# byteowlz/kokorox

Measured on NVIDIA B200. Metric: audio-seconds per second, higher is better.
Workload: dtype bf16

## Files before the change

kokorox_b200/csrc/kernels.h:

```cpp
#pragma once
#include "common.h"
#include <cuda_bf16.h>

namespace kkx {

enum Act : int { ACT_NONE = 0, ACT_LRELU = 1, ACT_SNAKE = 2, ACT_GELU_NEW = 3 };

struct ConvArgs {
  const float* in = nullptr; int ldi = 0;
  const int* in_off = nullptr; const int* in_len = nullptr;
  const int* m_len = nullptr; int max_m = 0; int B = 1;
  long long sum_m = 0;
  const float* w = nullptr; const float* bias = nullptr;
  int Ci = 0, Co = 0, ks = 1, dil = 1, pad = 0, stride = 1;
  const float* pscale = nullptr; const float* pshift = nullptr; int pld = 0;
  int pact = ACT_NONE; float pslope = 0.f; const float* palpha = nullptr;
  float* out = nullptr; int ldo = 0; int ocol = 0; const int* out_off = nullptr;
  int ors = 1, oro = 0;
  int eact = ACT_NONE;
  const float* res = nullptr; int ldr = 0; int rcol = 0; const int* res_off = nullptr;
  int res_shift = 0;
  float oscale = 1.f; int accumulate = 0;
};
void launch_conv_f32(const ConvArgs& a, cudaStream_t st);
// ... 54 lines not shown
void launch_im2col_bf16(const float* in, int ldi, int C, int ks, int stride, int pad, void* out, int Cpad,
                        int rows_total, const int* in_off, const int* in_len, const int* out_off,
                        const int* out_len, int B, int max_out_len, cudaStream_t st, int force_generic = 0);
void launch_pool_up_bf16(const float* in, int ldi, const float* scale, const float* shift, float slope,
                         const float* w, const float* bias, int C, void* out, int Cpad, int rows_total,
                         const int* in_off, const int* in_len, const int* out_off, int B, int max_len,
                         cudaStream_t st);

struct ArbConvArgs {
  const void* x = nullptr; int in_bf16 = 0;
  const float* scale = nullptr; const float* shift = nullptr;
  const float* alpha = nullptr;
  const void* tmB = nullptr;
  int C = 0, ks = 1, dil = 1, pad = 0;
  const int* off = nullptr; const int* len = nullptr;
  const int* tile_start = nullptr;
  int B = 1; int total_tiles = 0; long long sum_m = 0;
  const float* bias = nullptr;
  __nv_bfloat16* out_bf16 = nullptr;
  float* out_f32 = nullptr;
  const float* res = nullptr; float oscale = 1.f; int accumulate = 0;
  int res_bf16 = 0;
  float* part = nullptr; int nchunk = 0;
  long long* timing = nullptr;
  int debug = 0;
  int post = 0, cout = 0, ldo = 0; float slope = 0.f;
};
int arb_tile_rows(int C, int ks);
bool arb_conv_supported(int C, int ks, int dil, int B);
void launch_arb_conv(const ArbConvArgs& a, cudaStream_t st);
// ... 115 lines not shown
```

kokorox_b200/csrc/kernels_arb.cu:

```cuda
#include "kernels.h"
#include "tc_ptx.cuh"
#include <type_traits>
#include <cstdlib>

namespace kkx {

namespace {

#ifdef KKX_ARB_TIMING
#define TIM_DECL(n) long long tim_acc[n] = {0}; long long tim_last = clock64(); const bool tim_on = a.timing && blockIdx.x == 0
#define TICK(slot) do { if (tim_on) { const long long now_ = clock64(); tim_acc[slot] += now_ - tim_last; tim_last = now_; } } while (0)
#define TIM_FLUSH(base, n) do { if (tim_on) for (int i_ = 0; i_ < (n); i_++) atomicAdd(reinterpret_cast<unsigned long long*>(a.timing) + (base) + i_, (unsigned long long)tim_acc[i_]); } while (0)
#else
#define TIM_DECL(n)
#define TICK(slot)
#define TIM_FLUSH(base, n)
#endif

#ifdef KKX_EXPERIMENTS
#define ARB_DBG(a, bit) ((a).debug & (bit))
#else
#define ARB_DBG(a, bit) (0)
#endif

constexpr int kArbThreads = 512;
constexpr int kArbMaxB = 512;

template <int BN, int MSUB, bool T>
struct ArbCfg {
  static constexpr int KCH = BN / 64;
  static constexpr int RA = MSUB * 128 + 56;
  static constexpr uint32_t A_SLOT = RA * 128;
  static constexpr int NA = (BN == 128 && (!T || MSUB == 4)) ? 2 : 3;
  static constexpr uint32_t B_STAGE = BN * 128;
  static constexpr int NB = (T && MSUB == 4) ? 4 : (BN == 128) ? 6 : 3;
  static constexpr int PITCH = 36;
  static constexpr uint32_t STG = T ? 0 : 2 * 128 * PITCH * 4;
  static constexpr uint32_t STAT = 4 * BN * 2 * 4;
  static constexpr uint32_t COEF = 3 * BN * 4;
  static constexpr int NBAR = 2 * NA + 2 * NB + 4;
  static constexpr uint32_t SMEM = NA * A_SLOT + NB * B_STAGE + STG + STAT + COEF + NBAR * 8 + 16 + (3 * kArbMaxB + 2) * 4 + 1024;
  static_assert(A_SLOT % 1024 == 0, "A slot must keep the 1024-byte swizzle alignment");
};

__device__ __forceinline__ uint32_t pack_bf16(float lo, float hi) {
  __nv_bfloat162 p = __floats2bfloat162_rn(lo, hi);
  return *reinterpret_cast<uint32_t*>(&p);
}

struct TileCur {
  int b, mt;
  __device__ __forceinline__ void init(const int* ts, int B, int tile) {
    int lo = 0, hi = B;
    while (hi - lo > 1) {
      const int mid = (lo + hi) >> 1;
      if (ts[mid] <= tile) lo = mid; else hi = mid;
    }
    b = lo; mt = tile - ts[lo];
  }
  __device__ __forceinline__ void next(const int* ts) {
    mt++;
    while (ts[b] + mt >= ts[b + 1]) { b++; mt = 0; if (ts[b] < 0) break; }
  }
};

template <int BN, int MSUB, bool CONV2, bool T, bool POST = false, int SB = 0, bool PB = false>
__global__ void __launch_bounds__(kArbThreads, 1) arb_conv_kernel(const __grid_constant__ CUtensorMap tmB, ArbConvArgs a) {
  static_assert(SB == 0 || (!POST && (CONV2 || SB == 1)), "stream-bf16 variants: conv1 SB=1, conv2 SB=1 (bf16 out) / SB=2 (fp32 out)");
  static_assert(!PB || (T && !CONV2 && !POST && SB == 0 && MSUB == 2), "balanced-producer variant: conv1, transposed accumulator, fp32 input");
  constexpr bool XIN_BF = CONV2 || SB != 0;
  constexpr bool OUT_BF = !CONV2 || SB == 1;
  static_assert(!T || (BN == 128 && (MSUB == 2 || MSUB == 4)), "transposed mode: C = 128, 256- or 512-row tiles");
  static_assert(!POST || (T && !CONV2 && MSUB == 2), "post variant: transposed accumulator, fp32 input");
  constexpr int NBUF = (T && MSUB == 4) ? 1 : 2;
  constexpr int NEW = PB ? 4 : 8;
  constexpr int NPW = PB ? 8 : 14 - NEW;
  constexpr int kProdThreads = NPW * 32;
  constexpr int kProdRows = kProdThreads / 8;
  using Cfg = ArbCfg<BN, MSUB, T>;
  constexpr int KCH = Cfg::KCH, NA = Cfg::NA, NB = Cfg::NB, PITCH = Cfg::PITCH;
  constexpr int MT = MSUB * 128;
  extern __shared__ uint8_t smem_raw[];
// ... 1 lines not shown
  uint8_t* const gbase = smem_raw + (base - smem_u32(smem_raw));
  const uint32_t a_base = base;
  const uint32_t b_base = a_base + NA * Cfg::A_SLOT;
  const uint32_t stg_base = b_base + NB * Cfg::B_STAGE;
  const uint32_t stat_base = stg_base + Cfg::STG;
  const uint32_t coef_base = stat_base + Cfg::STAT;
  const uint32_t bar_base = coef_base + Cfg::COEF;
  const uint32_t tmem_slot = bar_base + Cfg::NBAR * 8;
  const uint32_t ts_base = tmem_slot + 16;
  auto fullA = [&](int s) { return bar_base + s * 8; };
  auto emptyA = [&](int s) { return bar_base + (NA + s) * 8; };
  auto fullB = [&](int s) { return bar_base + (2 * NA + s) * 8; };
  auto emptyB = [&](int s) { return bar_base + (2 * NA + NB + s) * 8; };
  auto tfull = [&](int j) { return bar_base + (2 * NA + 2 * NB + j) * 8; };
  auto tempty = [&](int j) { return bar_base + (2 * NA + 2 * NB + 2 + j) * 8; };
  int* const s_ts = reinterpret_cast<int*>(gbase + (ts_base - base));
  int* const s_len = s_ts + (kArbMaxB + 2);
  int* const s_off = s_len + kArbMaxB;

  const int warp = threadIdx.x >> 5, lane = threadIdx.x & 31;
  const int B = a.B;
#pragma unroll 1
  for (int i = threadIdx.x; i <= B + 1; i += kArbThreads) s_ts[i] = i <= B ? a.tile_start[i] : -1;
#pragma unroll 1
  for (int i = threadIdx.x; i < B; i += kArbThreads) { s_len[i] = a.len[i]; s_off[i] = a.off[i]; }

  if (warp == 0 && lane == 0) {
    asm volatile("prefetch.tensormap [%0];" ::"l"(&tmB) : "memory");
    for (int s = 0; s < NA; s++) { mbar_init(fullA(s), kProdThreads / 32); mbar_init(emptyA(s), 1); }
    for (int s = 0; s < NB; s++) { mbar_init(fullB(s), 1); mbar_init(emptyB(s), 1); }
    for (int j = 0; j < 2; j++) { mbar_init(tfull(j), 1); mbar_init(tempty(j), NEW); }
    asm volatile("fence.mbarrier_init.release.cluster;" ::: "memory");
    asm volatile("fence.proxy.async.shared::cta;" ::: "memory");
  }
  if (warp == 1) {
    asm volatile("tcgen05.alloc.cta_group::1.sync.aligned.shared::cta.b32 [%0], %1;" ::"r"(tmem_slot), "r"(512u) : "memory");
    asm volatile("tcgen05.relinquish_alloc_permit.cta_group::1.sync.aligned;" ::: "memory");
  }
  tc_fence_before();
  __syncthreads();
  tc_fence_after();
  uint32_t tmem_base;
  asm volatile("ld.shared.b32 %0, [%1];" : "=r"(tmem_base) : "r"(tmem_slot) : "memory");

// ... 372 lines not shown
          body(e + 1, rv1, std::true_type{});
        }
        continue;
      }
#pragma unroll 1
      for (int e = 0; e < E; e += 2) {
        body(e, rv0, std::false_type{});
        body(e + 1, rv1, std::false_type{});
      }
    }
    TIM_FLUSH(8, 9);
  } else if (warp < 2 + NEW + NPW) {
    const int pt = threadIdx.x - (2 + NEW) * 32;
    const int cg = pt & 7;
    const int rl = pt >> 3;
    constexpr int GP = PB ? 3 : 4;
    constexpr int GR = GP * kProdRows;
    const int ra_used = MT + 2 * pad;
    const int ngc = (ra_used + GR - 1) / GR;
    float* const coef = reinterpret_cast<float*>(gbase + (coef_base - base));
    const int F = (t_end - t_begin) * KCH * ngc;
    using Raw = typename std::conditional<XIN_BF, uint4, float4>::type;
    constexpr int RPP = XIN_BF ? 1 : 2;
    constexpr int XE = XIN_BF ? 2 : 4;
    const uint32_t sw = (uint32_t)rl * 128u + (uint32_t)((cg ^ (rl & 7)) << 4);

    TileCur lc; int l_c = 0, l_g = 0;
    TileCur sc_; int s_c = 0, s_g = 0, gA = 0, coef_b = -1;
    if (F > 0) { lc.init(s_ts, B, t_begin); sc_ = lc; }
    float2 cA[4], cB[4], cI[4];
#ifdef KKX_ARB_TIMING
    long long tim_acc[5] = {0}; long long tim_last = clock64();
    const bool tim_on = a.timing && blockIdx.x == 0 && warp == 10 && lane == 0;
#endif

    auto issue = [&](Raw (&rb)[GP][RPP]) {
      const int L = s_len[lc.b];
      const int row = lc.mt * MT - pad + l_g * GR + rl;
      const int rloc = l_g * GR + rl;
      const char* xp = reinterpret_cast<const char*>(a.x) + ((size_t)(s_off[lc.b] + row) * BN + (l_c * 64 + cg * 8)) * XE;
#pragma unroll
      for (int p = 0; p < GP; p++) {
        if ((unsigned)(row + p * kProdRows) < (unsigned)L && rloc + p * kProdRows < ra_used && !ARB_DBG(a, 1)) {
#pragma unroll
          for (int v = 0; v < RPP; v++) {
            const char* gp = xp + (size_t)p * kProdRows * BN * XE + v * 16;
            if (ARB_DBG(a, 16)) {
              uint4 t;
              asm volatile("ld.global.L1::no_allocate.v4.u32 {%0, %1, %2, %3}, [%4];" : "=r"(t.x), "=r"(t.y), "=r"(t.z), "=r"(t.w) : "l"(gp));
              rb[p][v] = *reinterpret_cast<Raw*>(&t);
            } else rb[p][v] = *reinterpret_cast<const Raw*>(gp);
          }
        }
      }
      if (++l_g == ngc) { l_g = 0; if (++l_c == KCH) { l_c = 0; lc.next(s_ts); } }
    };
    auto process = [&](Raw (&rb)[GP][RPP]) {
      const int b = sc_.b;
      const int sa = gA % NA;
      if (s_g == 0) {
        if (!POST && b != coef_b) {
          asm volatile("bar.sync 3, %0;" ::"n"(kProdThreads) : "memory");
          for (int ch = pt; ch < BN; ch += kProdThreads) {
            const float al = a.alpha[ch], s = a.scale[(size_t)b * BN + ch], h = a.shift[(size_t)b * BN + ch];
            coef[ch] = al * s; coef[BN + ch] = al * h; coef[2 * BN + ch] = 1.0f / al;
          }
          asm volatile("bar.sync 3, %0;" ::"n"(kProdThreads) : "memory");
          coef_b = b;
        }
        const float* cp = coef + s_c * 64 + cg * 8;
#pragma unroll
        for (int e = 0; !POST && e < 4; e += 2) {
          const float4 t0 = *reinterpret_cast<const float4*>(cp + 2 * e);
          const float4 t1 = *reinterpret_cast<const float4*>(cp + BN + 2 * e);
          const float4 t2 = *reinterpret_cast<const float4*>(cp + 2 * BN + 2 * e);
          cA[e] = make_float2(t0.x, t0.y); cA[e + 1] = make_float2(t0.z, t0.w);
          cB[e] = make_float2(t1.x, t1.y); cB[e + 1] = make_float2(t1.z, t1.w);
          cI[e] = make_float2(t2.x, t2.y); cI[e + 1] = make_float2(t2.z, t2.w);
        }
        TICK(1);
        mbar_wait(emptyA(sa), (((uint32_t)(gA / NA)) & 1u) ^ 1u);
        TICK(2);
      }
      const int L = s_len[b];
      const int row = sc_.mt * MT - pad + s_g * GR + rl;
      const int rloc = s_g * GR + rl;
      uint8_t* const sp = gbase + (a_base - base) + (size_t)sa * Cfg::A_SLOT + (size_t)(s_g * GR) * 128 + sw;
#pragma unroll
      for (int p = 0; p < GP; p++) {
        const uint32_t inmask = (unsigned)(row + p * kProdRows) < (unsigned)L ? 0xFFFFFFFFu : 0u;
        float2 xv[4];
        if (XIN_BF) {
          const uint4 raw = *reinterpret_cast<const uint4*>(&rb[p][0]);
          xv[0] = make_float2(__uint_as_float(raw.x << 16), __uint_as_float(raw.x & 0xFFFF0000u));
          xv[1] = make_float2(__uint_as_float(raw.y << 16), __uint_as_float(raw.y & 0xFFFF0000u));
          xv[2] = make_float2(__uint_as_float(raw.z << 16), __uint_as_float(raw.z & 0xFFFF0000u));
          xv[3] = make_float2(__uint_as_float(raw.w << 16), __uint_as_float(raw.w & 0xFFFF0000u));
        } else {
          const float4 f0 = *reinterpret_cast<const float4*>(&rb[p][0]);
          const float4 f1 = *reinterpret_cast<const float4*>(&rb[p][RPP - 1]);
          xv[0] = make_float2(f0.x, f0.y); xv[1] = make_float2(f0.z, f0.w);
          xv[2] = make_float2(f1.x, f1.y); xv[3] = make_float2(f1.z, f1.w);
        }
        uint32_t pw[4];
#pragma unroll
        for (int e = 0; e < 4; e++) {
          if (POST) {
            const float2 lx = __fmul2_rn(xv[e], make_float2(a.slope, a.slope));
            pw[e] = pack_bf16(fmaxf(xv[e].x, lx.x), fmaxf(xv[e].y, lx.y)) & inmask;
            continue;
          }
          if (ARB_DBG(a, 4)) { pw[e] = pack_bf16(xv[e].x, xv[e].y) & inmask; continue; }
          const float2 u = __ffma2_rn(xv[e], cA[e], cB[e]);
          const float2 sn = make_float2(__sinf(u.x), __sinf(u.y));
          const float2 y = __fmul2_rn(__ffma2_rn(sn, sn, u), cI[e]);
          pw[e] = pack_bf16(y.x, y.y) & inmask;
        }
        const uint4 pk = make_uint4(pw[0], pw[1], pw[2], pw[3]);
        if (rloc + p * kProdRows < ra_used) *reinterpret_cast<uint4*>(sp + p * kProdRows * 128) = pk;
      }
      TICK(3);
      if (++s_g == ngc) {
        asm volatile("fence.proxy.async.shared::cta;" ::: "memory");
        __syncwarp();
        if (lane == 0) asm volatile("mbarrier.arrive.shared::cta.b64 _, [%0];" ::"r"(fullA(sa)) : "memory");
        s_g = 0; gA++;
        if (++s_c == KCH) { s_c = 0; sc_.next(s_ts); }
      }
    };

    Raw bufA[GP][RPP], bufB[GP][RPP];
#pragma unroll
    for (int p = 0; p < GP; p++)
#pragma unroll
      for (int v = 0; v < RPP; v++) { bufA[p][v] = Raw(); bufB[p][v] = Raw(); }
    if (F > 0) issue(bufA);
#pragma unroll 1
    for (int f = 0; f < F; f += 2) {
      if (f + 1 < F) issue(bufB);
      TICK(0);
      process(bufA);
      if (f + 1 >= F) break;
      if (f + 2 < F) issue(bufA);
      TICK(0);
      process(bufB);
    }
    TIM_FLUSH(20, 5);
  }
  tc_fence_before();
  __syncthreads();
  if (warp == 1) {
    tc_fence_after();
    asm volatile("tcgen05.dealloc.cta_group::1.sync.aligned.b32 %0, %1;" ::"r"(tmem_base), "r"(512u) : "memory");
  }
}

template <int BN, int MSUB, bool CONV2, bool T, bool POST = false, int SB = 0, bool PB = false>
void launch_arb_t(const ArbConvArgs& a, cudaStream_t st) {
  using Cfg = ArbCfg<BN, MSUB, T>;
  static DevOnce once;
  int dev = 0;
  cudaGetDevice(&dev);
  once.run(dev, [] { KKX_CUDA(cudaFuncSetAttribute(arb_conv_kernel<BN, MSUB, CONV2, T, POST, SB, PB>, cudaFuncAttributeMaxDynamicSharedMemorySize, (int)Cfg::SMEM)); });
  const int nsm = device_sm_count(dev);
  const int grid = a.total_tiles < nsm ? a.total_tiles : nsm;
  arb_conv_kernel<BN, MSUB, CONV2, T, POST, SB, PB><<<grid, kArbThreads, Cfg::SMEM, st>>>(*reinterpret_cast<const CUtensorMap*>(a.tmB), a);
}

}

static int arb_variant(int C, int ks) {
  static const bool no_t = env_flag("KKX_ARB_NOT", false);
  static const bool use_512 = env_flag("KKX_ARB_512", false);
  if (C != 128 || no_t) return 0;
  return (ks >= 7 && use_512) ? 2 : 1;
}
int arb_tile_rows(int C, int ks) { return C == 128 ? (arb_variant(C, ks) == 2 ? 512 : 256) : 128; }

bool arb_conv_supported(int C, int ks, int dil, int B) {
  return (C == 128 || C == 256) && ks >= 1 && dil >= 1 && dil * (ks - 1) <= 50 && (ks & 1) && B <= kArbMaxB;
}
// ... 62 lines not shown
```

kokorox_b200/csrc/model_forward.cu:

```cuda
#include "model.h"
#include <algorithm>
#include <cmath>
#include <cstdlib>

namespace kkx {

namespace {
long long* g_arb_timing = nullptr;
long long* arb_timing_buf() {
  static const bool on = env_flag("KKX_ARB_TIMING", false);
  if (!on) return nullptr;
  if (!g_arb_timing) {
    KKX_CUDA(cudaMalloc(&g_arb_timing, 128 * sizeof(long long)));
    KKX_CUDA(cudaMemset(g_arb_timing, 0, 128 * sizeof(long long)));
  }
  return g_arb_timing;
}
ConvArgs gemm_args(const Level& L, const float* in, int ldi, int K, const float* w, const float* bias,
                   int N, float* out, int ldo, int ocol) {
  ConvArgs a;
  a.in = in; a.ldi = ldi; a.in_off = L.d_off; a.in_len = L.d_len;
  a.m_len = L.d_len; a.max_m = L.max_len; a.B = L.B; a.sum_m = L.sum_len;
  a.w = w; a.bias = bias; a.Ci = K; a.Co = N;
  a.out = out; a.ldo = ldo; a.ocol = ocol; a.out_off = L.d_off;
// ... 4 lines not shown
void arb_timing_dump() {
  if (!g_arb_timing) return;
  attention_timing_dump();
  long long h[128];
  cudaDeviceSynchronize();
  cudaMemcpy(h, g_arb_timing, sizeof h, cudaMemcpyDeviceToHost);
  cudaMemset(g_arb_timing, 0, sizeof h);
  fprintf(stderr, "[tf32x3 timing, CTA 0 of every launch] (Mcycles) TMA wait_empty %.2f issue %.2f | MMA wait_full %.2f wait_ring %.2f issue %.2f |"
          " EPI wait_chain %.2f drain %.2f wait_final %.2f final %.2f\n", h[100] / 1e6, h[101] / 1e6, h[104] / 1e6, h[105] / 1e6, h[106] / 1e6,
          h[108] / 1e6, h[109] / 1e6, h[110] / 1e6, h[111] / 1e6);
  const char* nm[4] = {"conv1 C128", "conv2 C128", "conv1 C256", "conv2 C256"};
  for (int v = 0; v < 3; v++) {
    const long long* t = h + v * 32;
    fprintf(stderr, "[arb timing %s] (Mcycles)  TMA wait %.2f issue %.2f | MMA wait_tempty %.2f wait_fullA %.2f wait_fullB %.2f issue %.2f |"
            " EPI wait_tfull %.2f tmem_ld %.2f barA %.2f sts %.2f barB %.2f compute+store %.2f fetch %.2f stats %.2f tile %.2f |"
            " PROD issue %.2f coef %.2f wait_emptyA %.2f transform %.2f mov+arrive %.2f\n", nm[v],
            t[0] / 1e6, t[1] / 1e6, t[4] / 1e6, t[5] / 1e6, t[6] / 1e6, t[7] / 1e6, t[8] / 1e6, t[9] / 1e6, t[10] / 1e6, t[11] / 1e6,
            t[12] / 1e6, t[13] / 1e6, t[14] / 1e6, t[15] / 1e6, t[16] / 1e6, t[20] / 1e6, t[21] / 1e6, t[22] / 1e6, t[23] / 1e6, t[24] / 1e6);
  }
}

void Model::tc_conv(Arena& A, const void* abuf, int rows_total, const TcW& w, int dil, int pad, const Level& Lin,
                    const Level& Lm, const float* bias, float* out, int ldo, int ocol, const Level& Lout, int ors,
                    int oro, const float* res, int ldr, const Level* Lres, int res_shift, float oscale,
                    bool accumulate) {
  (void)A;
  alignas(64) unsigned char tmA[128];
  if (g_dry_run) return;
  make_tmap_bf16(tmA, abuf, w.Cpad, rows_total, w.Cpad, 128);
  TcConvArgs a;
  a.tmA = tmA; a.tmB = w.tmap;
  a.Cpad = w.Cpad; a.Ci = w.Ci; a.Co = w.Co; a.ks = w.ks; a.dil = dil; a.pad = pad;
  a.in_off = Lin.d_off; a.m_len = Lm.d_len; a.max_m = Lm.max_len; a.B = Lm.B; a.sum_m = Lm.sum_len;
// ... 379 lines not shown
                const void* x_bf16) {
  (void)r;
  cudaStream_t st = cur_;
  const int B = L.B, C = w.c, k = w.k;
  const int nch = (L.max_len + kStatRows - 1) / kStatRows;
  float* part = A.alloc<float>((size_t)B * nch * 2 * C);
  float* sc = A.alloc<float>((size_t)B * C);
  float* sh = A.alloc<float>((size_t)B * C);
  const int dil[3] = {1, 3, 5};
  const float* cur = x;
  const bool tc = opt.precision == 1;
  void* abuf = tc ? A.alloc_bytes((size_t)L.rows * w.t1[0].Cpad * 2) : nullptr;
  static const bool fused_ok = env_flag("KKX_ARB_FUSED", true);
  if (tc && fused_ok && arb_conv_supported(C, k, 5, B)) {
    ArbConvArgs base;
    base.C = C; base.ks = k; base.off = L.d_off; base.len = L.d_len; base.B = B; base.sum_m = L.sum_len;
    const int trows = arb_tile_rows(C, k);
    base.tile_start = trows == 512 ? L.d_tiles512 : trows == 256 ? L.d_tiles256 : L.d_tiles128;
    base.total_tiles = trows == 512 ? L.ntiles512 : trows == 256 ? L.ntiles256 : L.ntiles128;
    base.scale = sc; base.shift = sh; base.nchunk = nch;
    const bool sb = use_stream_bf16(C, k, B);
    void* xb0 = nullptr;
    if (sb && !x_bf16) xb0 = A.alloc_bytes((size_t)L.rows * C * 2);
    if (!part_x) launch_colstats(cur, C, C, part, L.d_off, L.d_len, B, L.max_len, st, xb0);
    else if (sb && !x_bf16) throw ArgError("arb: a bf16 stream with caller-provided statistics needs the bf16 input too");
    const void* curb = sb ? (x_bf16 ? x_bf16 : xb0) : nullptr;
    long long* tim = arb_timing_buf();
    static const int tim_ks = env_int("KKX_ARB_TIMING_KS", 0);
    if (tim_ks && tim_ks != k) tim = nullptr;
    for (int j = 0; j < 3; j++) {
      launch_adain_coef(j == 0 && part_x ? part_x : part, C, L.max_len, L.d_len, sty, sld, w.s1[j], 1e-5f, sc, sh, B, st);
// ... 368 lines not shown
      const bool sb1 = use_stream_bf16(128, 3, B) && use_stream_bf16(128, 7, B) && use_stream_bf16(128, 11, B);
      xb = sb1 ? A.alloc_bytes((size_t)G120.rows * 128 * 2) : nullptr;
      launch_add_rows_stats(x1, xs1, x1, 128, px, G120.d_off, G120.d_len, B, G120.max_len, st, xb);
    } else {
      launch_add_rows(x1, xs1, x1, 128, G120.d_off, G120.d_len, B, G120.max_len, st);
    }
    for (int j = 0; j < 3; j++)
      arb(r, A, W.res[3 + j], x1, G120, sty_dec, W.sty_dec_n, w1, t1, acc1, 1.0f / 3.0f, j > 0, px, xb);
  }
  capture("gen.stage.1", acc1, 128, 0, 128, G120, b0);

  float* cp = A.alloc<float>((size_t)G120.rows * 24);
  static const bool post_fused = env_flag("KKX_POST_FUSED", true);
  if (opt.precision == 1 && post_fused && arb_conv_supported(128, 7, 1, B)) {
    ArbConvArgs pc;
    pc.C = 128; pc.ks = 7; pc.dil = 1; pc.pad = 3; pc.off = G120.d_off; pc.len = G120.d_len; pc.B = B;
    pc.sum_m = G120.sum_len; pc.tile_start = G120.d_tiles256; pc.total_tiles = G120.ntiles256;
    pc.x = acc1; pc.in_bf16 = 0; pc.tmB = W.t_post_arb.tmap; pc.bias = W.post_b128;
    pc.out_f32 = cp; pc.post = 1; pc.cout = 22; pc.ldo = 24; pc.slope = 0.01f;
    launch_arb_conv(pc, st);
  } else if (opt.precision == 1) {
    void* pb = A.alloc_bytes((size_t)G120.rows * 128 * 2);
    launch_apply_bf16(acc1, 128, 128, nullptr, nullptr, ACT_LRELU, 0.01f, nullptr, pb, 128, G120.rows, G120.d_off,
                      G120.d_len, B, G120.max_len, st);
    tc_conv(A, pb, G120.rows, W.t_post, 1, 3, G120, G120, W.post_b, cp, 24, 0, G120, 1, 0, nullptr, 0, nullptr, 0, 1.f, false);
  } else {
    ConvArgs c = gemm_args(G120, acc1, 128, 128, W.post_w, W.post_b, 22, cp, 24, 0);
    c.ks = 7; c.pad = 3; c.pact = ACT_LRELU; c.pslope = 0.01f;
    launch_conv_f32(c, st);
  }
  capture("conv_post", cp, 24, 0, 22, G120, b0);
// ... 19 lines not shown
```

kokorox_b200/csrc/tc_ptx.cuh:

```cuda
#pragma once
#include <cuda.h>
#include <cuda_bf16.h>
#include <stdint.h>

namespace kkx {

__device__ __forceinline__ uint32_t smem_u32(const void* p) { return (uint32_t)__cvta_generic_to_shared(p); }

__device__ __forceinline__ void mbar_init(uint32_t bar, uint32_t count) {
  asm volatile("mbarrier.init.shared::cta.b64 [%0], %1;" ::"r"(bar), "r"(count));
}
__device__ __forceinline__ void mbar_expect_tx(uint32_t bar, uint32_t bytes) {
  asm volatile("mbarrier.arrive.expect_tx.shared::cta.b64 _, [%0], %1;" ::"r"(bar), "r"(bytes) : "memory");
}
__device__ __forceinline__ void mbar_wait(uint32_t bar, uint32_t parity) {
  asm volatile(
      "{\n\t.reg .pred p;\n\t"
      "WAIT_%=:\n\t"
      "mbarrier.try_wait.parity.shared::cta.b64 p, [%0], %1, %2;\n\t"
      "@p bra DONE_%=;\n\t"
      "bra WAIT_%=;\n\t"
      "DONE_%=:\n\t}" ::"r"(bar), "r"(parity), "r"(0x989680u) : "memory");
}
__device__ __forceinline__ void tma_load_2d(uint32_t dst, const void* tmap, int c0, int c1, uint32_t bar) {
  asm volatile(
      "cp.async.bulk.tensor.2d.shared::cluster.global.mbarrier::complete_tx::bytes [%0], [%1, {%3, %4}], [%2];"
      ::"r"(dst), "l"(tmap), "r"(bar), "r"(c0), "r"(c1) : "memory");
}
__device__ __forceinline__ void tma_load_2d_mc(uint32_t dst, const void* tmap, int c0, int c1, uint32_t bar, uint16_t mask) {
  asm volatile(
      "cp.async.bulk.tensor.2d.shared::cluster.global.mbarrier::complete_tx::bytes.multicast::cluster [%0], [%1, {%3, %4}], [%2], %5;"
      ::"r"(dst), "l"(tmap), "r"(bar), "r"(c0), "r"(c1), "h"(mask) : "memory");
}
__device__ __forceinline__ uint32_t cluster_ctarank() {
  uint32_t r;
  asm volatile("mov.u32 %0, %%cluster_ctarank;" : "=r"(r));
  return r;
// ... 99 lines not shown
```

kokorox_b200/csrc/testapi.cu:

```cuda
#include "../../include/kkx_test.h"
#include "kernels.h"
#include "model.h"
#include <algorithm>
#include <cstring>
#include <limits>
#include <string>
#include <vector>

using namespace kkx;
static thread_local std::string t_err;

namespace {
struct DevBuf {
  void* p = nullptr;
  DevBuf(const void* host, size_t bytes) {
    KKX_CUDA(cudaMalloc(&p, bytes ? bytes : 4));
    if (host && bytes) KKX_CUDA(cudaMemcpy(p, host, bytes, cudaMemcpyHostToDevice));
  }
  ~DevBuf() { if (p) cudaFree(p); }
  template <class T> T* as() { return static_cast<T*>(p); }
};
template <class F> int run(int device, F&& f) {
  try {
    int n = 0;
// ... 473 lines not shown
static inline uint16_t host_bf16(float f) {
  uint32_t u; memcpy(&u, &f, 4);
  return (uint16_t)((u + 0x7FFFu + ((u >> 16) & 1u)) >> 16);
}

}

static int arb_conv_test(int device, const float* x, int B, const int* lens, int C, int in_bf16,
                         const float* scale, const float* shift, const float* alpha, const float* w,
                         const float* bias, int ks, int dil, const float* res, int res_bf16, float oscale,
                         int accumulate, int want_bf16, float* out, float* sums, int desc_mode) {
  return run(device, [&] {
    if (!arb_conv_supported(C, ks, dil, B)) throw ArgError("kkx_test_arb_conv: unsupported shape");
    std::vector<int> off(B), tiles(B + 1, 0);
    const int MT = arb_tile_rows(C, ks);
    int o = kGapRows, maxL = 0; long long sumL = 0;
    for (int b = 0; b < B; b++) {
      off[b] = o; o = (o + lens[b] + kGapRows + 7) & ~7;
      tiles[b + 1] = tiles[b] + (lens[b] + MT - 1) / MT;
      maxL = std::max(maxL, lens[b]); sumL += lens[b];
    }
    const int rows = o;
    const float qnan = std::numeric_limits<float>::quiet_NaN();
    std::vector<float> hx((size_t)rows * C, qnan), hres((size_t)rows * C, qnan), hout((size_t)rows * C, qnan);
    size_t src = 0;
    for (int b = 0; b < B; b++) {
      memcpy(hx.data() + (size_t)off[b] * C, x + src * C, (size_t)lens[b] * C * 4);
      if (res) memcpy(hres.data() + (size_t)off[b] * C, res + src * C, (size_t)lens[b] * C * 4);
      memcpy(hout.data() + (size_t)off[b] * C, out + src * C, (size_t)lens[b] * C * 4);
      src += lens[b];
    }
    std::vector<uint16_t> hxb;
    if (in_bf16) { hxb.resize(hx.size()); for (size_t i = 0; i < hx.size(); i++) hxb[i] = host_bf16(hx[i]); }
    std::vector<uint16_t> hw((size_t)C * ks * C);
    for (size_t i = 0; i < hw.size(); i++) hw[i] = host_bf16(w[i]);
    DevBuf dx(in_bf16 ? (const void*)hxb.data() : (const void*)hx.data(), hx.size() * (in_bf16 ? 2 : 4));
    DevBuf dw(hw.data(), hw.size() * 2), db(bias, C * 4), dsc(scale, (size_t)B * C * 4), dsh(shift, (size_t)B * C * 4);
    std::vector<uint16_t> hresb;
    if (res && res_bf16) { hresb.resize(hres.size()); for (size_t i = 0; i < hres.size(); i++) hresb[i] = host_bf16(hres[i]); }
    DevBuf dal(alpha, C * 4), dres(res ? (res_bf16 ? (const void*)hresb.data() : (const void*)hres.data()) : nullptr,
                                   res ? hres.size() * (res_bf16 ? 2 : 4) : 0);
    DevBuf dout(hout.data(), hout.size() * 4), doutb(nullptr, hout.size() * 2);
    KKX_CUDA(cudaMemset(doutb.p, 0xFF, hout.size() * 2));
    const int nchunk = (maxL + 127) / 128;
    DevBuf dpart(nullptr, (size_t)B * nchunk * 2 * C * 4);
    KKX_CUDA(cudaMemset(dpart.p, 0, (size_t)B * nchunk * 2 * C * 4));
    DevBuf doff(off.data(), B * 4), dlen(lens, B * 4), dts(tiles.data(), (B + 1) * 4);
    alignas(64) unsigned char tmB[128];
    make_tmap_bf16(tmB, dw.p, (long long)ks * C, C, (long long)ks * C, tc_box_n(C));
    ArbConvArgs a;
    a.x = dx.p; a.in_bf16 = in_bf16; a.scale = dsc.as<float>(); a.shift = dsh.as<float>(); a.alpha = dal.as<float>();
    a.tmB = tmB; a.C = C; a.ks = ks; a.dil = dil; a.pad = dil * (ks - 1) / 2;
    a.off = doff.as<int>(); a.len = dlen.as<int>(); a.tile_start = dts.as<int>(); a.B = B; a.total_tiles = tiles[B];
    a.sum_m = sumL; a.bias = db.as<float>();
    a.out_bf16 = want_bf16 ? doutb.as<__nv_bfloat16>() : nullptr;
    a.out_f32 = want_bf16 ? nullptr : dout.as<float>();
    a.res = res ? dres.as<float>() : nullptr; a.res_bf16 = res ? res_bf16 : 0; a.oscale = oscale; a.accumulate = accumulate;
    a.part = sums ? dpart.as<float>() : nullptr; a.nchunk = nchunk; (void)desc_mode;
    launch_arb_conv(a, 0);
    KKX_CUDA(cudaDeviceSynchronize());
    if (want_bf16) {
      std::vector<uint16_t> hb(hout.size());
      KKX_CUDA(cudaMemcpy(hb.data(), doutb.p, hb.size() * 2, cudaMemcpyDeviceToHost));
      for (size_t i = 0; i < hb.size(); i++) { uint32_t u = (uint32_t)hb[i] << 16; memcpy(&hout[i], &u, 4); }
    } else {
      KKX_CUDA(cudaMemcpy(hout.data(), dout.p, hout.size() * 4, cudaMemcpyDeviceToHost));
    }
    src = 0;
// ... 38 lines not shown
```

Baseline: 10460.

## Load bf16 conv input halos via TMA into smem before in-place snake transform

For bf16-input variants of the fused snake+conv kernel, producer warps no longer issue per-thread global loads. A single thread now issues TMA 2D loads of the haloed input tile into the A slot, tracked by a new per-slot raw barrier. Producers then transform the data in place in shared memory and signal the MMA warp. This frees producer registers and load-issue slots and lets the copy overlap other work. In exchange it adds a tensor map per launch, an extra barrier wait per chunk, slightly larger A slots for 512-row tiles, and a dependency on the buffer row count for out-of-bounds handling.

```diff
diff --git a/kokorox_b200/csrc/kernels.h b/kokorox_b200/csrc/kernels.h
--- a/kokorox_b200/csrc/kernels.h
+++ b/kokorox_b200/csrc/kernels.h
@@ -92,6 +92,7 @@
   const void* tmB = nullptr;
   int C = 0, ks = 1, dil = 1, pad = 0;
   const int* off = nullptr; const int* len = nullptr;
+  int rows = 0;
   const int* tile_start = nullptr;
   int B = 1; int total_tiles = 0; long long sum_m = 0;
   const float* bias = nullptr;
diff --git a/kokorox_b200/csrc/kernels_arb.cu b/kokorox_b200/csrc/kernels_arb.cu
--- a/kokorox_b200/csrc/kernels_arb.cu
+++ b/kokorox_b200/csrc/kernels_arb.cu
@@ -29,7 +29,7 @@
 template <int BN, int MSUB, bool T>
 struct ArbCfg {
   static constexpr int KCH = BN / 64;
-  static constexpr int RA = MSUB * 128 + 56;
+  static constexpr int RA = MSUB * 128 + (MSUB == 4 ? 64 : 56);
   static constexpr uint32_t A_SLOT = RA * 128;
   static constexpr int NA = (BN == 128 && (!T || MSUB == 4)) ? 2 : 3;
   static constexpr uint32_t B_STAGE = BN * 128;
@@ -38,10 +38,19 @@
   static constexpr uint32_t STG = T ? 0 : 2 * 128 * PITCH * 4;
   static constexpr uint32_t STAT = 4 * BN * 2 * 4;
   static constexpr uint32_t COEF = 3 * BN * 4;
-  static constexpr int NBAR = 2 * NA + 2 * NB + 4;
+  static constexpr int NBAR = 3 * NA + 2 * NB + 4;
   static constexpr uint32_t SMEM = NA * A_SLOT + NB * B_STAGE + STG + STAT + COEF + NBAR * 8 + 16 + (3 * kArbMaxB + 2) * 4 + 1024;
   static_assert(A_SLOT % 1024 == 0, "A slot must keep the 1024-byte swizzle alignment");
+  static_assert(SMEM <= 232448, "shared memory of one block");
 };
+
+__host__ __device__ constexpr int arb_halo_box(int ra, int RA) {
+  for (int n = 1; n <= 8; n++) {
+    const int box = ((ra + n - 1) / n + 7) & ~7;
+    if (box <= 256 && n * box <= RA) return box;
+  }
+  return 0;
+}
 
 __device__ __forceinline__ uint32_t pack_bf16(float lo, float hi) {
   __nv_bfloat162 p = __floats2bfloat162_rn(lo, hi);
@@ -65,7 +74,8 @@
 };
 
 template <int BN, int MSUB, bool CONV2, bool T, bool POST = false, int SB = 0, bool PB = false>
-__global__ void __launch_bounds__(kArbThreads, 1) arb_conv_kernel(const __grid_constant__ CUtensorMap tmB, ArbConvArgs a) {
+__global__ void __launch_bounds__(kArbThreads, 1) arb_conv_kernel(const __grid_constant__ CUtensorMap tmB,
+                                                                   const __grid_constant__ CUtensorMap tmX, ArbConvArgs a) {
   static_assert(SB == 0 || (!POST && (CONV2 || SB == 1)), "stream-bf16 variants: conv1 SB=1, conv2 SB=1 (bf16 out) / SB=2 (fp32 out)");
   static_assert(!PB || (T && !CONV2 && !POST && SB == 0 && MSUB == 2), "balanced-producer variant: conv1, transposed accumulator, fp32 input");
   constexpr bool XIN_BF = CONV2 || SB != 0;
@@ -97,6 +107,7 @@
   auto emptyB = [&](int s) { return bar_base + (2 * NA + NB + s) * 8; };
   auto tfull = [&](int j) { return bar_base + (2 * NA + 2 * NB + j) * 8; };
   auto tempty = [&](int j) { return bar_base + (2 * NA + 2 * NB + 2 + j) * 8; };
+  auto rawA = [&](int s) { return bar_base + (2 * NA + 2 * NB + 4 + s) * 8; };
   int* const s_ts = reinterpret_cast<int*>(gbase + (ts_base - base));
   int* const s_len = s_ts + (kArbMaxB + 2);
   int* const s_off = s_len + kArbMaxB;
@@ -110,7 +121,8 @@
 
   if (warp == 0 && lane == 0) {
     asm volatile("prefetch.tensormap [%0];" ::"l"(&tmB) : "memory");
-    for (int s = 0; s < NA; s++) { mbar_init(fullA(s), kProdThreads / 32); mbar_init(emptyA(s), 1); }
+    if (XIN_BF) asm volatile("prefetch.tensormap [%0];" ::"l"(&tmX) : "memory");
+    for (int s = 0; s < NA; s++) { mbar_init(fullA(s), kProdThreads / 32); mbar_init(emptyA(s), 1); mbar_init(rawA(s), 1); }
     for (int s = 0; s < NB; s++) { mbar_init(fullB(s), 1); mbar_init(emptyB(s), 1); }
     for (int j = 0; j < 2; j++) { mbar_init(tfull(j), 1); mbar_init(tempty(j), NEW); }
     asm volatile("fence.mbarrier_init.release.cluster;" ::: "memory");
@@ -513,138 +525,201 @@
     const int pt = threadIdx.x - (2 + NEW) * 32;
     const int cg = pt & 7;
     const int rl = pt >> 3;
-    constexpr int GP = PB ? 3 : 4;
-    constexpr int GR = GP * kProdRows;
     const int ra_used = MT + 2 * pad;
-    const int ngc = (ra_used + GR - 1) / GR;
     float* const coef = reinterpret_cast<float*>(gbase + (coef_base - base));
-    const int F = (t_end - t_begin) * KCH * ngc;
-    using Raw = typename std::conditional<XIN_BF, uint4, float4>::type;
-    constexpr int RPP = XIN_BF ? 1 : 2;
-    constexpr int XE = XIN_BF ? 2 : 4;
     const uint32_t sw = (uint32_t)rl * 128u + (uint32_t)((cg ^ (rl & 7)) << 4);
-
-    TileCur lc; int l_c = 0, l_g = 0;
-    TileCur sc_; int s_c = 0, s_g = 0, gA = 0, coef_b = -1;
-    if (F > 0) { lc.init(s_ts, B, t_begin); sc_ = lc; }
+    TileCur sc_; int s_c = 0, coef_b = -1;
     float2 cA[4], cB[4], cI[4];
 #ifdef KKX_ARB_TIMING
-    long long tim_acc[5] = {0}; long long tim_last = clock64();
+    long long tim_acc[7] = {0}; long long tim_last = clock64();
     const bool tim_on = a.timing && blockIdx.x == 0 && warp == 10 && lane == 0;
 #endif
-
-    auto issue = [&](Raw (&rb)[GP][RPP]) {
-      const int L = s_len[lc.b];
-      const int row = lc.mt * MT - pad + l_g * GR + rl;
-      const int rloc = l_g * GR + rl;
-      const char* xp = reinterpret_cast<const char*>(a.x) + ((size_t)(s_off[lc.b] + row) * BN + (l_c * 64 + cg * 8)) * XE;
-#pragma unroll
-      for (int p = 0; p < GP; p++) {
-        if ((unsigned)(row + p * kProdRows) < (unsigned)L && rloc + p * kProdRows < ra_used && !ARB_DBG(a, 1)) {
-#pragma unroll
-          for (int v = 0; v < RPP; v++) {
-            const char* gp = xp + (size_t)p * kProdRows * BN * XE + v * 16;
-            if (ARB_DBG(a, 16)) {
-              uint4 t;
-              asm volatile("ld.global.L1::no_allocate.v4.u32 {%0, %1, %2, %3}, [%4];" : "=r"(t.x), "=r"(t.y), "=r"(t.z), "=r"(t.w) : "l"(gp));
-              rb[p][v] = *reinterpret_cast<Raw*>(&t);
-            } else rb[p][v] = *reinterpret_cast<const Raw*>(gp);
-          }
-        }
-      }
-      if (++l_g == ngc) { l_g = 0; if (++l_c == KCH) { l_c = 0; lc.next(s_ts); } }
+    auto chunk_coef = [&]() {
+      const int b = sc_.b;
+      if (!POST && b != coef_b) {
+        asm volatile("bar.sync 3, %0;" ::"n"(kProdThreads) : "memory");
+        for (int ch = pt; ch < BN; ch += kProdThreads) {
+          const float al = a.alpha[ch], s = a.scale[(size_t)b * BN + ch], h = a.shift[(size_t)b * BN + ch];
+          coef[ch] = al * s; coef[BN + ch] = al * h; coef[2 * BN + ch] = 1.0f / al;
+        }
+        asm volatile("bar.sync 3, %0;" ::"n"(kProdThreads) : "memory");
+        coef_b = b;
+      }
+      const float* cp = coef + s_c * 64 + cg * 8;
+#pragma unroll
+      for (int e = 0; !POST && e < 4; e += 2) {
+        const float4 t0 = *reinterpret_cast<const float4*>(cp + 2 * e);
+        const float4 t1 = *reinterpret_cast<const float4*>(cp + BN + 2 * e);
+        const float4 t2 = *reinterpret_cast<const float4*>(cp + 2 * BN + 2 * e);
+        cA[e] = make_float2(t0.x, t0.y); cA[e + 1] = make_float2(t0.z, t0.w);
+        cB[e] = make_float2(t1.x, t1.y); cB[e + 1] = make_float2(t1.z, t1.w);
+        cI[e] = make_float2(t2.x, t2.y); cI[e + 1] = make_float2(t2.z, t2.w);
+      }
     };
-    auto process = [&](Raw (&rb)[GP][RPP]) {
-      const int b = sc_.b;
-      const int sa = gA % NA;
-      if (s_g == 0) {
-        if (!POST && b != coef_b) {
-          asm volatile("bar.sync 3, %0;" ::"n"(kProdThreads) : "memory");
-          for (int ch = pt; ch < BN; ch += kProdThreads) {
-            const float al = a.alpha[ch], s = a.scale[(size_t)b * BN + ch], h = a.shift[(size_t)b * BN + ch];
-            coef[ch] = al * s; coef[BN + ch] = al * h; coef[2 * BN + ch] = 1.0f / al;
-          }
-          asm volatile("bar.sync 3, %0;" ::"n"(kProdThreads) : "memory");
-          coef_b = b;
-        }
-        const float* cp = coef + s_c * 64 + cg * 8;
-#pragma unroll
-        for (int e = 0; !POST && e < 4; e += 2) {
-          const float4 t0 = *reinterpret_cast<const float4*>(cp + 2 * e);
-          const float4 t1 = *reinterpret_cast<const float4*>(cp + BN + 2 * e);
-          const float4 t2 = *reinterpret_cast<const float4*>(cp + 2 * BN + 2 * e);
-          cA[e] = make_float2(t0.x, t0.y); cA[e + 1] = make_float2(t0.z, t0.w);
-          cB[e] = make_float2(t1.x, t1.y); cB[e + 1] = make_float2(t1.z, t1.w);
-          cI[e] = make_float2(t2.x, t2.y); cI[e + 1] = make_float2(t2.z, t2.w);
-        }
+    auto transform8 = [&](const float2 (&xv)[4], uint32_t inmask) {
+      uint32_t pw[4];
+#pragma unroll
+      for (int e = 0; e < 4; e++) {
+        if (POST) {
+          const float2 lx = __fmul2_rn(xv[e], make_float2(a.slope, a.slope));
+          pw[e] = pack_bf16(fmaxf(xv[e].x, lx.x), fmaxf(xv[e].y, lx.y)) & inmask;
+          continue;
+        }
+        if (ARB_DBG(a, 4)) { pw[e] = pack_bf16(xv[e].x, xv[e].y) & inmask; continue; }
+        const float2 u = __ffma2_rn(xv[e], cA[e], cB[e]);
+        const float2 sn = make_float2(__sinf(u.x), __sinf(u.y));
+        const float2 y = __fmul2_rn(__ffma2_rn(sn, sn, u), cI[e]);
+        pw[e] = pack_bf16(y.x, y.y) & inmask;
+      }
+      return make_uint4(pw[0], pw[1], pw[2], pw[3]);
+    };
+    auto arrive_full = [&](int sa) {
+      asm volatile("fence.proxy.async.shared::cta;" ::: "memory");
+      __syncwarp();
+      if (lane == 0) asm volatile("mbarrier.arrive.shared::cta.b64 _, [%0];" ::"r"(fullA(sa)) : "memory");
+    };
+
+    if constexpr (XIN_BF) {
+      constexpr int GP = 4;
+      constexpr int GR = GP * kProdRows;
+      const int box = arb_halo_box(ra_used, Cfg::RA), nbox = (ra_used + box - 1) / box;
+      const int NC = (t_end - t_begin) * KCH;
+      TileCur lc; int l_c = 0, gL = 0;
+      if (NC > 0) { lc.init(s_ts, B, t_begin); sc_ = lc; }
+      auto issue = [&]() {
+        const int s = gL % NA;
+        const int row0 = s_off[lc.b] + lc.mt * MT - pad;
+        mbar_expect_tx(rawA(s), ARB_DBG(a, 1) ? 0u : (uint32_t)(nbox * box * 128));
+        if (!ARB_DBG(a, 1))
+          for (int i = 0; i < nbox; i++)
+            tma_load_2d(a_base + s * Cfg::A_SLOT + (uint32_t)(i * box * 128), &tmX, l_c * 64, row0 + i * box, rawA(s));
+        gL++;
+        if (++l_c == KCH) { l_c = 0; lc.next(s_ts); }
+      };
+      auto top_up = [&](int g) {
+        while (gL <= g) {
+          mbar_wait(emptyA(gL % NA), (((uint32_t)(gL / NA)) & 1u) ^ 1u);
+          TICK(5);
+          issue();
+        }
+        while (gL < NC && gL < g + NA && mbar_test(emptyA(gL % NA), (((uint32_t)(gL / NA)) & 1u) ^ 1u)) issue();
+      };
+#pragma unroll 1
+      for (int g = 0; g < NC; g++) {
+        const int sa = g % NA;
+        if (pt == 0) top_up(g);
+        TICK(0);
+        chunk_coef();
         TICK(1);
-        mbar_wait(emptyA(sa), (((uint32_t)(gA / NA)) & 1u) ^ 1u);
-        TICK(2);
-      }
-      const int L = s_len[b];
-      const int row = sc_.mt * MT - pad + s_g * GR + rl;
-      const int rloc = s_g * GR + rl;
-      uint8_t* const sp = gbase + (a_base - base) + (size_t)sa * Cfg::A_SLOT + (size_t)(s_g * GR) * 128 + sw;
-#pragma unroll
-      for (int p = 0; p < GP; p++) {
-        const uint32_t inmask = (unsigned)(row + p * kProdRows) < (unsigned)L ? 0xFFFFFFFFu : 0u;
-        float2 xv[4];
-        if (XIN_BF) {
-          const uint4 raw = *reinterpret_cast<const uint4*>(&rb[p][0]);
-          xv[0] = make_float2(__uint_as_float(raw.x << 16), __uint_as_float(raw.x & 0xFFFF0000u));
-          xv[1] = make_float2(__uint_as_float(raw.y << 16), __uint_as_float(raw.y & 0xFFFF0000u));
-          xv[2] = make_float2(__uint_as_float(raw.z << 16), __uint_as_float(raw.z & 0xFFFF0000u));
-          xv[3] = make_float2(__uint_as_float(raw.w << 16), __uint_as_float(raw.w & 0xFFFF0000u));
-        } else {
-          const float4 f0 = *reinterpret_cast<const float4*>(&rb[p][0]);
-          const float4 f1 = *reinterpret_cast<const float4*>(&rb[p][RPP - 1]);
-          xv[0] = make_float2(f0.x, f0.y); xv[1] = make_float2(f0.z, f0.w);
-          xv[2] = make_float2(f1.x, f1.y); xv[3] = make_float2(f1.z, f1.w);
-        }
-        uint32_t pw[4];
-#pragma unroll
-        for (int e = 0; e < 4; e++) {
-          if (POST) {
-            const float2 lx = __fmul2_rn(xv[e], make_float2(a.slope, a.slope));
-            pw[e] = pack_bf16(fmaxf(xv[e].x, lx.x), fmaxf(xv[e].y, lx.y)) & inmask;
-            continue;
-          }
-          if (ARB_DBG(a, 4)) { pw[e] = pack_bf16(xv[e].x, xv[e].y) & inmask; continue; }
-          const float2 u = __ffma2_rn(xv[e], cA[e], cB[e]);
-          const float2 sn = make_float2(__sinf(u.x), __sinf(u.y));
-          const float2 y = __fmul2_rn(__ffma2_rn(sn, sn, u), cI[e]);
-          pw[e] = pack_bf16(y.x, y.y) & inmask;
-        }
-        const uint4 pk = make_uint4(pw[0], pw[1], pw[2], pw[3]);
-        if (rloc + p * kProdRows < ra_used) *reinterpret_cast<uint4*>(sp + p * kProdRows * 128) = pk;
-      }
-      TICK(3);
-      if (++s_g == ngc) {
-        asm volatile("fence.proxy.async.shared::cta;" ::: "memory");
-        __syncwarp();
-        if (lane == 0) asm volatile("mbarrier.arrive.shared::cta.b64 _, [%0];" ::"r"(fullA(sa)) : "memory");
-        s_g = 0; gA++;
+        mbar_wait(rawA(sa), ((uint32_t)(g / NA)) & 1u);
+        TICK(6);
+        const int L = s_len[sc_.b];
+        const int row = sc_.mt * MT - pad + rl;
+        uint8_t* const sp = gbase + (a_base - base) + (size_t)sa * Cfg::A_SLOT + sw;
+#pragma unroll 1
+        for (int r0 = 0; r0 < ra_used; r0 += GR) {
+          uint4 raw[GP];
+#pragma unroll
+          for (int p = 0; p < GP; p++) {
+            raw[p] = make_uint4(0u, 0u, 0u, 0u);
+            if (r0 + p * kProdRows + rl < ra_used) raw[p] = *reinterpret_cast<const uint4*>(sp + (r0 + p * kProdRows) * 128);
+          }
+#pragma unroll
+          for (int p = 0; p < GP; p++) {
+            if (r0 + p * kProdRows >= ra_used) break;
+            const uint32_t inmask = (unsigned)(row + r0 + p * kProdRows) < (unsigned)L ? 0xFFFFFFFFu : 0u;
+            float2 xv[4];
+            xv[0] = make_float2(__uint_as_float(raw[p].x << 16), __uint_as_float(raw[p].x & 0xFFFF0000u));
+            xv[1] = make_float2(__uint_as_float(raw[p].y << 16), __uint_as_float(raw[p].y & 0xFFFF0000u));
+            xv[2] = make_float2(__uint_as_float(raw[p].z << 16), __uint_as_float(raw[p].z & 0xFFFF0000u));
+            xv[3] = make_float2(__uint_as_float(raw[p].w << 16), __uint_as_float(raw[p].w & 0xFFFF0000u));
+            const uint4 pk = transform8(xv, inmask);
+            if (r0 + p * kProdRows + rl < ra_used) *reinterpret_cast<uint4*>(sp + (r0 + p * kProdRows) * 128) = pk;
+          }
+          if (pt == 0) top_up(g);
+        }
+        TICK(3);
+        arrive_full(sa);
+        TICK(4);
         if (++s_c == KCH) { s_c = 0; sc_.next(s_ts); }
       }
-    };
-
-    Raw bufA[GP][RPP], bufB[GP][RPP];
-#pragma unroll
-    for (int p = 0; p < GP; p++)
-#pragma unroll
-      for (int v = 0; v < RPP; v++) { bufA[p][v] = Raw(); bufB[p][v] = Raw(); }
-    if (F > 0) issue(bufA);
-#pragma unroll 1
-    for (int f = 0; f < F; f += 2) {
-      if (f + 1 < F) issue(bufB);
-      TICK(0);
-      process(bufA);
-      if (f + 1 >= F) break;
-      if (f + 2 < F) issue(bufA);
-      TICK(0);
-      process(bufB);
+    } else {
+      constexpr int GP = PB ? 3 : 4;
+      constexpr int GR = GP * kProdRows;
+      const int ngc = (ra_used + GR - 1) / GR;
+      const int F = (t_end - t_begin) * KCH * ngc;
+      TileCur lc; int l_c = 0, l_g = 0;
+      int s_g = 0, gA = 0;
+      if (F > 0) { lc.init(s_ts, B, t_begin); sc_ = lc; }
+
+      auto issue = [&](float4 (&rb)[GP][2]) {
+        const int L = s_len[lc.b];
+        const int row = lc.mt * MT - pad + l_g * GR + rl;
+        const int rloc = l_g * GR + rl;
+        const float* xp = reinterpret_cast<const float*>(a.x) + (size_t)(s_off[lc.b] + row) * BN + (l_c * 64 + cg * 8);
+#pragma unroll
+        for (int p = 0; p < GP; p++) {
+          if ((unsigned)(row + p * kProdRows) < (unsigned)L && rloc + p * kProdRows < ra_used && !ARB_DBG(a, 1)) {
+#pragma unroll
+            for (int v = 0; v < 2; v++) {
+              const float* gp = xp + (size_t)p * kProdRows * BN + v * 4;
+              if (ARB_DBG(a, 16)) {
+                uint4 t;
+                asm volatile("ld.global.L1::no_allocate.v4.u32 {%0, %1, %2, %3}, [%4];" : "=r"(t.x), "=r"(t.y), "=r"(t.z), "=r"(t.w) : "l"(gp));
+                rb[p][v] = *reinterpret_cast<float4*>(&t);
+              } else rb[p][v] = *reinterpret_cast<const float4*>(gp);
+            }
+          }
+        }
+        if (++l_g == ngc) { l_g = 0; if (++l_c == KCH) { l_c = 0; lc.next(s_ts); } }
+      };
+      auto process = [&](float4 (&rb)[GP][2]) {
+        const int sa = gA % NA;
+        if (s_g == 0) {
+          chunk_coef();
+          TICK(1);
+          mbar_wait(emptyA(sa), (((uint32_t)(gA / NA)) & 1u) ^ 1u);
+          TICK(2);
+        }
+        const int L = s_len[sc_.b];
+        const int row = sc_.mt * MT - pad + s_g * GR + rl;
+        const int rloc = s_g * GR + rl;
+        uint8_t* const sp = gbase + (a_base - base) + (size_t)sa * Cfg::A_SLOT + (size_t)(s_g * GR) * 128 + sw;
+#pragma unroll
+        for (int p = 0; p < GP; p++) {
+          const uint32_t inmask = (unsigned)(row + p * kProdRows) < (unsigned)L ? 0xFFFFFFFFu : 0u;
+          float2 xv[4];
+          xv[0] = make_float2(rb[p][0].x, rb[p][0].y); xv[1] = make_float2(rb[p][0].z, rb[p][0].w);
+          xv[2] = make_float2(rb[p][1].x, rb[p][1].y); xv[3] = make_float2(rb[p][1].z, rb[p][1].w);
+          const uint4 pk = transform8(xv, inmask);
+          if (rloc + p * kProdRows < ra_used) *reinterpret_cast<uint4*>(sp + p * kProdRows * 128) = pk;
+        }
+        TICK(3);
+        if (++s_g == ngc) {
+          arrive_full(sa);
+          s_g = 0; gA++;
+          if (++s_c == KCH) { s_c = 0; sc_.next(s_ts); }
+        }
+      };
+
+      float4 bufA[GP][2], bufB[GP][2];
+#pragma unroll
+      for (int p = 0; p < GP; p++)
+#pragma unroll
+        for (int v = 0; v < 2; v++) { bufA[p][v] = float4(); bufB[p][v] = float4(); }
+      if (F > 0) issue(bufA);
+#pragma unroll 1
+      for (int f = 0; f < F; f += 2) {
+        if (f + 1 < F) issue(bufB);
+        TICK(0);
+        process(bufA);
+        if (f + 1 >= F) break;
+        if (f + 2 < F) issue(bufA);
+        TICK(0);
+        process(bufB);
+      }
     }
-    TIM_FLUSH(20, 5);
+    TIM_FLUSH(20, 7);
   }
   tc_fence_before();
   __syncthreads();
@@ -663,7 +738,13 @@
   once.run(dev, [] { KKX_CUDA(cudaFuncSetAttribute(arb_conv_kernel<BN, MSUB, CONV2, T, POST, SB, PB>, cudaFuncAttributeMaxDynamicSharedMemorySize, (int)Cfg::SMEM)); });
   const int nsm = device_sm_count(dev);
   const int grid = a.total_tiles < nsm ? a.total_tiles : nsm;
-  arb_conv_kernel<BN, MSUB, CONV2, T, POST, SB, PB><<<grid, kArbThreads, Cfg::SMEM, st>>>(*reinterpret_cast<const CUtensorMap*>(a.tmB), a);
+  CUtensorMap tmX{};
+  if (CONV2 || SB != 0) {
+    const int box = arb_halo_box(MSUB * 128 + 2 * a.pad, Cfg::RA);
+    if (a.rows <= 0 || box == 0) throw ArgError("launch_arb_conv: bf16 input needs its buffer's row count");
+    make_tmap_bf16(&tmX, a.x, BN, a.rows, BN, box);
+  }
+  arb_conv_kernel<BN, MSUB, CONV2, T, POST, SB, PB><<<grid, kArbThreads, Cfg::SMEM, st>>>(*reinterpret_cast<const CUtensorMap*>(a.tmB), tmX, a);
 }
 
 }
diff --git a/kokorox_b200/csrc/model_forward.cu b/kokorox_b200/csrc/model_forward.cu
--- a/kokorox_b200/csrc/model_forward.cu
+++ b/kokorox_b200/csrc/model_forward.cu
@@ -42,9 +42,10 @@
     const long long* t = h + v * 32;
     fprintf(stderr, "[arb timing %s] (Mcycles)  TMA wait %.2f issue %.2f | MMA wait_tempty %.2f wait_fullA %.2f wait_fullB %.2f issue %.2f |"
             " EPI wait_tfull %.2f tmem_ld %.2f barA %.2f sts %.2f barB %.2f compute+store %.2f fetch %.2f stats %.2f tile %.2f |"
-            " PROD issue %.2f coef %.2f wait_emptyA %.2f transform %.2f mov+arrive %.2f\n", nm[v],
+            " PROD issue %.2f coef %.2f wait_emptyA %.2f transform %.2f arrive %.2f wait_slot_free %.2f wait_raw_landed %.2f\n", nm[v],
             t[0] / 1e6, t[1] / 1e6, t[4] / 1e6, t[5] / 1e6, t[6] / 1e6, t[7] / 1e6, t[8] / 1e6, t[9] / 1e6, t[10] / 1e6, t[11] / 1e6,
-            t[12] / 1e6, t[13] / 1e6, t[14] / 1e6, t[15] / 1e6, t[16] / 1e6, t[20] / 1e6, t[21] / 1e6, t[22] / 1e6, t[23] / 1e6, t[24] / 1e6);
+            t[12] / 1e6, t[13] / 1e6, t[14] / 1e6, t[15] / 1e6, t[16] / 1e6, t[20] / 1e6, t[21] / 1e6, t[22] / 1e6, t[23] / 1e6, t[24] / 1e6,
+            t[25] / 1e6, t[26] / 1e6);
   }
 }
 
@@ -454,7 +455,7 @@
   static const bool fused_ok = env_flag("KKX_ARB_FUSED", true);
   if (tc && fused_ok && arb_conv_supported(C, k, 5, B)) {
     ArbConvArgs base;
-    base.C = C; base.ks = k; base.off = L.d_off; base.len = L.d_len; base.B = B; base.sum_m = L.sum_len;
+    base.C = C; base.ks = k; base.off = L.d_off; base.len = L.d_len; base.rows = L.rows; base.B = B; base.sum_m = L.sum_len;
     const int trows = arb_tile_rows(C, k);
     base.tile_start = trows == 512 ? L.d_tiles512 : trows == 256 ? L.d_tiles256 : L.d_tiles128;
     base.total_tiles = trows == 512 ? L.ntiles512 : trows == 256 ? L.ntiles256 : L.ntiles128;
@@ -853,7 +854,7 @@
   static const bool post_fused = env_flag("KKX_POST_FUSED", true);
   if (opt.precision == 1 && post_fused && arb_conv_supported(128, 7, 1, B)) {
     ArbConvArgs pc;
-    pc.C = 128; pc.ks = 7; pc.dil = 1; pc.pad = 3; pc.off = G120.d_off; pc.len = G120.d_len; pc.B = B;
+    pc.C = 128; pc.ks = 7; pc.dil = 1; pc.pad = 3; pc.off = G120.d_off; pc.len = G120.d_len; pc.rows = G120.rows; pc.B = B;
     pc.sum_m = G120.sum_len; pc.tile_start = G120.d_tiles256; pc.total_tiles = G120.ntiles256;
     pc.x = acc1; pc.in_bf16 = 0; pc.tmB = W.t_post_arb.tmap; pc.bias = W.post_b128;
     pc.out_f32 = cp; pc.post = 1; pc.cout = 22; pc.ldo = 24; pc.slope = 0.01f;
diff --git a/kokorox_b200/csrc/tc_ptx.cuh b/kokorox_b200/csrc/tc_ptx.cuh
--- a/kokorox_b200/csrc/tc_ptx.cuh
+++ b/kokorox_b200/csrc/tc_ptx.cuh
@@ -21,6 +21,14 @@
       "@p bra DONE_%=;\n\t"
       "bra WAIT_%=;\n\t"
       "DONE_%=:\n\t}" ::"r"(bar), "r"(parity), "r"(0x989680u) : "memory");
+}
+__device__ __forceinline__ bool mbar_test(uint32_t bar, uint32_t parity) {
+  uint32_t ok;
+  asm volatile(
+      "{\n\t.reg .pred p;\n\t"
+      "mbarrier.test_wait.parity.shared::cta.b64 p, [%1], %2;\n\t"
+      "selp.u32 %0, 1, 0, p;\n\t}" : "=r"(ok) : "r"(bar), "r"(parity) : "memory");
+  return ok != 0;
 }
 __device__ __forceinline__ void tma_load_2d(uint32_t dst, const void* tmap, int c0, int c1, uint32_t bar) {
   asm volatile(
diff --git a/kokorox_b200/csrc/testapi.cu b/kokorox_b200/csrc/testapi.cu
--- a/kokorox_b200/csrc/testapi.cu
+++ b/kokorox_b200/csrc/testapi.cu
@@ -511,13 +511,13 @@
     if (!arb_conv_supported(C, ks, dil, B)) throw ArgError("kkx_test_arb_conv: unsupported shape");
     std::vector<int> off(B), tiles(B + 1, 0);
     const int MT = arb_tile_rows(C, ks);
-    int o = kGapRows, maxL = 0; long long sumL = 0;
+    int o = 0, maxL = 0; long long sumL = 0;
     for (int b = 0; b < B; b++) {
       off[b] = o; o = (o + lens[b] + kGapRows + 7) & ~7;
       tiles[b + 1] = tiles[b] + (lens[b] + MT - 1) / MT;
       maxL = std::max(maxL, lens[b]); sumL += lens[b];
     }
-    const int rows = o;
+    const int rows = off[B - 1] + lens[B - 1];
     const float qnan = std::numeric_limits<float>::quiet_NaN();
     std::vector<float> hx((size_t)rows * C, qnan), hres((size_t)rows * C, qnan), hout((size_t)rows * C, qnan);
     size_t src = 0;
@@ -548,7 +548,7 @@
     ArbConvArgs a;
     a.x = dx.p; a.in_bf16 = in_bf16; a.scale = dsc.as<float>(); a.shift = dsh.as<float>(); a.alpha = dal.as<float>();
     a.tmB = tmB; a.C = C; a.ks = ks; a.dil = dil; a.pad = dil * (ks - 1) / 2;
-    a.off = doff.as<int>(); a.len = dlen.as<int>(); a.tile_start = dts.as<int>(); a.B = B; a.total_tiles = tiles[B];
+    a.off = doff.as<int>(); a.len = dlen.as<int>(); a.rows = rows; a.tile_start = dts.as<int>(); a.B = B; a.total_tiles = tiles[B];
     a.sum_m = sumL; a.bias = db.as<float>();
     a.out_bf16 = want_bf16 ? doutb.as<__nv_bfloat16>() : nullptr;
     a.out_f32 = want_bf16 ? nullptr : dout.as<float>();
```

New measurement: 10550 (median of 6 runs). No clear change (+0.8%).
